# NJU-3DV/Relightable3DGaussian

Measured on AMD Instinct MI355X. Metric: train iters/s, synthetic lego-like 800x800, 300000 Gaussians (stage-2 hot path), higher is better.
Workload: dtype f32; 1 GPU; stage-2 train iteration (fused glue kernels + one-launch Adam): shading fwd/bwd (K=64) + rasterize fwd (S=16) + loss + rasterize bwd + Adam; 1 view/rank/step, 300000 Gaussians, 800x800, num_rendered~1755016; parallelism=dp1

## Files before the change

### relightable3dgaussian_amd/csrc/capi_rasterizer.hip

```cpp
#include "capi_internal.hpp"

#include <mutex>
#include <vector>

namespace r3dg {

GeometryLayout GeometryLayout::make(size_t P)
{
    GeometryLayout L;
    size_t o = 0;
    auto take = [&](size_t bytes) { size_t r = o; o = align_up(o + bytes, 256); return r; };
    L.depths = take(P * 4);
    L.clamped = take(P * 3);
    L.radii = take(P * 4);
    L.means2D = take(P * 8);
    L.cov3D = take(P * 24);
    L.conic_opacity = take(P * 16);
    L.rgb = take(P * 12);
    L.tiles_touched = take(P * 4);
    L.point_offsets = take(P * 4);
    L.block_sums = take(((P + 255) / 256 + 1) * 4);
    L.total = take(8);
    L.splat = take(P * 64);
    L.bytes = o;
// ... 96 lines not shown
        if (!g_ticket_pool.empty()) {
            ForwardTicket* t = g_ticket_pool.back();
            g_ticket_pool.pop_back();
            return t;
        }
    }
    ForwardTicket* t = new ForwardTicket();
    R3DG_HIP(hipEventCreateWithFlags(&t->ready, hipEventDisableTiming));
    R3DG_HIP(hipEventCreateWithFlags(&t->ordered, hipEventDisableTiming));
    R3DG_HIP(hipHostMalloc((void**)&t->host_total, sizeof(unsigned long long), hipHostMallocDefault));
    return t;
}
static void ticket_release(ForwardTicket* t)
{
    std::lock_guard<std::mutex> lk(g_ticket_mutex);
    g_ticket_pool.push_back(t);
}

static int enqueue_ordering(ForwardTicket* t, hipStream_t stream, int R)
{
    const ForwardArgs& a = t->a;
    const GeometryLayout& G = t->v.G;
    const ImageLayout& I = t->v.I;
    const bool debug = a.debug != 0;
    const int P = a.P, gx = t->v.gx, gy = t->v.gy, T = (int)t->v.T;
    char *gbuf = t->gbuf, *ibuf = t->ibuf;
    int* radii_p = t->radii_p;
    float* g_depths = (float*)(gbuf + G.depths);
    float* g_means2D = (float*)(gbuf + G.means2D);
    uint32_t* g_tiles = (uint32_t*)(gbuf + G.tiles_touched);
    uint32_t* g_block = (uint32_t*)(gbuf + G.block_sums);
    const bool direct = direct_binning_usable((long long)t->v.T);
    if (a.capacity >= 0 && !direct) {
        set_error("rasterize_forward (bounded): needs the direct tile binning and at most 16384 tiles: ask r3dg_bounded_forward_supported(width, height) first");
        return R3DG_EINVAL;
    }
    BinningLayout B = BinningLayout::make((size_t)R);
    char* bbuf = t->fused_front ? t->bbuf : (char*)a.binning_alloc(a.user, B.bytes);
    t->bbuf = bbuf;
    if (!bbuf) { set_error("rasterize_forward: binning resize callback returned NULL"); return R3DG_EALLOC; }
    uint64_t* keys_u = (uint64_t*)(bbuf + B.keys_unsorted);
    uint64_t* keys = (uint64_t*)(bbuf + B.keys);
    uint32_t* vals_u = (uint32_t*)(bbuf + B.vals_unsorted);
    uint32_t* vals = (uint32_t*)(bbuf + B.vals);
    t->point_list = vals;

    uint32_t* ranges = (uint32_t*)(ibuf + I.ranges);
    uint32_t* order = (uint32_t*)(ibuf + I.tile_order);
    uint32_t* big_list = (uint32_t*)(ibuf + I.big_list);
    uint32_t* big_count = (uint32_t*)(ibuf + I.big_count);
    if (direct) {
        uint32_t* tile_counts = (uint32_t*)(bbuf + B.sort_temp);
        StageTimer t_dup(stream, ST_DUPKEYS);
        launch_tile_binning(stream, P, T, g_means2D, g_depths, radii_p, g_tiles, g_block, gx, gy, tile_counts, tile_counts + T,
                            ranges, (uint32_t*)(gbuf + G.point_offsets), keys_u, (unsigned long long*)(gbuf + G.total), a.capacity,
                            a.overflow_flag, a.overflow_count, t->fused_front, order, tile_sort_small_cap(), big_list, big_count);
        check_launch(stream, debug, "tile_binning");
        t_dup.stop();
        StageTimer t_sort(stream, ST_SORT);
        if (!t->fused_front) {
            launch_tile_order(stream, T, ranges, order, tile_sort_small_cap(), big_list, big_count);
            check_launch(stream, debug, "tile_order");
        }
        launch_tile_sort(stream, T, order, ranges, big_list, big_count, keys, vals, keys_u, true);
        check_launch(stream, debug, "tile_sort");
        t_sort.stop();
        return R3DG_OK;
    }
    StageTimer t_dup(stream, ST_DUPKEYS);
    launch_duplicate_with_keys(stream, P, g_means2D, g_depths, g_tiles, g_block, (uint32_t*)(gbuf + G.point_offsets),
                               keys_u, vals_u, radii_p, gx, gy);
    check_launch(stream, debug, "duplicate_with_keys");
    t_dup.stop();
    const int bit = (int)higher_msb((uint32_t)T);
    StageTimer t_sort(stream, ST_SORT);
    if (opt(R3DG_OPT_TILE_BINNING)) {
        sort_pairs_range(stream, (size_t)R, keys_u, vals_u, keys, vals, 32, 32 + bit, bbuf + B.sort_temp, debug,
                         false);
        R3DG_HIP(hipMemsetAsync(ranges, 0, (size_t)T * 8, stream));
        launch_identify_tile_ranges(stream, R, keys, ranges);
        check_launch(stream, debug, "identify_tile_ranges");
        launch_tile_order(stream, T, ranges, order, tile_sort_small_cap(), big_list, big_count);
        check_launch(stream, debug, "tile_order");
        launch_tile_sort(stream, T, order, ranges, big_list, big_count, keys, vals, keys_u, false);
        check_launch(stream, debug, "tile_sort");
        t_sort.stop();
    } else {
        sort_pairs(stream, (size_t)R, keys_u, vals_u, keys, vals, 32 + bit, bbuf + B.sort_temp, debug);
        t_sort.stop();

        StageTimer t_rng(stream, ST_RANGES);
        R3DG_HIP(hipMemsetAsync(ranges, 0, (size_t)T * 8, stream));
        launch_identify_tile_ranges(stream, R, keys, ranges);
        check_launch(stream, debug, "identify_tile_ranges");
        t_rng.stop();
        if (opt(R3DG_OPT_TILE_ORDER)) {
            launch_tile_order(stream, T, ranges, order, 0u, nullptr, nullptr);
            check_launch(stream, debug, "tile_order");
        }
    }
    return R3DG_OK;
}

static void render_tiles(const ForwardTicket* t, hipStream_t stream)
{
    const ForwardArgs& a = t->a;
    const GeometryLayout& G = t->v.G;
    const ImageLayout& I = t->v.I;
    const bool debug = a.debug != 0;
    StageTimer t_rf(stream, ST_RENDER_FWD);
    launch_render_forward(stream, a.width, a.height, a.S,
                          opt(R3DG_OPT_TILE_ORDER) ? (uint32_t*)(t->ibuf + I.tile_order) : nullptr,
                          (uint32_t*)(t->ibuf + I.ranges), t->point_list, (const float*)(t->gbuf + G.splat), a.features,
                          (float*)(t->ibuf + I.final_T), (uint32_t*)(t->ibuf + I.n_contrib), a.background, a.out_color,
                          a.out_opacity, a.out_depth, a.out_feature, a.out_weights);
    check_launch(stream, debug, "render_forward");
// ... 387 lines not shown
```

### relightable3dgaussian_amd/csrc/launchers.hpp

```cpp
#pragma once
#include "common.hpp"

namespace r3dg {

__attribute__((visibility("hidden"))) int persistent_cus();

void release_gradient_records();
void launch_mark_visible(hipStream_t s, int P, const float* means3D, const float* vm, uint8_t* present);
void launch_preprocess(hipStream_t s, int P, int D, int M, const float* means3D, const float* scales, float scale_modifier,
                       const float* rotations, const float* opacities, const float* shs, uint8_t* clamped,
                       const float* cov3D_precomp, const float* colors_precomp, const float* vm, const float* pm,
                       const float* cam_pos, int W, int H, float tan_fovx, float tan_fovy, float focal_x, float focal_y,
                       int* radii, float* means2D, float* depths, float* cov3Ds, float* rgb, float* conic_opacity,
                       float* splat, int gx, int gy, uint32_t* tiles_touched, uint32_t* block_sums,
                       unsigned long long* total, bool scan_now, uint32_t* zero_words, int zero_n);
void launch_duplicate_with_keys(hipStream_t s, int P, const float* means2D, const float* depths,
                                const uint32_t* tiles_touched, const uint32_t* block_offsets, uint32_t* point_offsets,
                                uint64_t* keys, uint32_t* values, const int* radii, int gx, int gy);
void launch_identify_tile_ranges(hipStream_t s, int L, const uint64_t* keys, uint32_t* ranges);
void launch_tile_order(hipStream_t s, int T, const uint32_t* ranges, uint32_t* order, uint32_t small_cap, uint32_t* big_list,
                       uint32_t* big_count);
void launch_render_forward(hipStream_t s, int W, int H, int S, const uint32_t* tile_order, const uint32_t* ranges,
                           const uint32_t* point_list, const float* splat, const float* features, float* final_T,
                           uint32_t* n_contrib, const float* bg, float* out_color, float* out_opacity, float* out_depth,
// ... 110 lines not shown
                      float* dL_dpbr, float* dL_ddiffuse, float* block_absmax, float* light_l1_sum);
void launch_s2_activate_backward(hipStream_t s, int P, const float* xyz, const float* scaling_raw, const float* rotation_raw,
                                 const float* opacity_raw, const float* normal_raw, const float* base_raw,
                                 const float* rough_raw, const float* viewmatrix, const float* campos,
                                 const float* dL_dfeatures, const float* dL_dbase_shade, const float* dL_drough_shade,
                                 const float* dL_dviewdirs, const float* dL_dscales, const float* dL_drot,
                                 const float* dL_dopacity, const float* dL_dmeans3D, float* g_xyz, float* g_scaling,
                                 float* g_rotation, float* g_opacity, float* g_normal, float* g_base, float* g_rough, int He,
                                 int We, const float* env_raw, const float* env, float* dL_denv, float w_tv,
                                 float* g_env_raw, float* tv_sum, int consume);
void launch_s2_loss(hipStream_t s, int HW, const float* image, const float* opacity, const float* feature,
                    const float* pseudo_normal, const int* n_contrib, const float* gt, const float* bg,
                    const float* image_mask, float w_l1, float w_pbr, float w_normal, const float* extra_dimage,
                    const float* extra_dsrgb, float* dL_dimage, float* dL_dopacity, float* dL_dfeature, float* sums,
                    int sparse);
void launch_s2_smooth_forward(hipStream_t s, int W, int H, const float* opacity, const float* feature, const int* n_contrib,
                              const float* gt, const float* image_mask, float w_base, float w_rough, float w_light,
                              float* scratch, float* sums3);
void launch_s2_smooth_fused(hipStream_t s, int W, int H, const float* opacity, const float* feature, const int* n_contrib,
                            const float* gt, const float* image_mask, float w_base, float w_rough, float w_light,
                            int accumulate_normal, float* dL_dopacity, float* dL_dfeature, float* sums3);
void launch_s2_smooth_backward(hipStream_t s, int W, int H, const float* opacity, const float* feature, const int* n_contrib,
                               const float* image_mask, const float* scratch, int has_base, int has_rough, int has_light,
                               int accumulate_normal, float* dL_dopacity, float* dL_dfeature);
void launch_s2_pbr_srgb(hipStream_t s, int HW, const float* opacity, const float* feature, const int* n_contrib,
                        const float* bg, float* srgb);
void launch_s2_normals_srgb(hipStream_t s, int W, int H, const float* vm, float focal_x, float focal_y, float cx, float cy,
                            const float* opacity, const float* depths, float* normals, float* surface_xyz,
                            const float* feature, const int* n_contrib, const float* bg, float* srgb);
void launch_ssim_forward(hipStream_t s, int W, int H, int C, int n_images, const float* const* x, const float* y,
                         float* const* partials, float* const* sum);
void launch_ssim_backward(hipStream_t s, int W, int H, int C, int n_images, const float* const* x, const float* y,
                          float* const* partials, const float* scale, float* const* grad_x);
void launch_adam(hipStream_t s, int n_groups, const r3dg_adam_group* groups, float beta1, float beta2, float eps, int step,
                 float grad_scale, const float* skip_flag);
void launch_s1_pack(hipStream_t s, int P, const float* xyz, const float* viewmatrix, const float* normal, float* features);
void launch_s1_edge(hipStream_t s, int W, int H, const float* feature, const float* opacity, const int* n_contrib,
                    const float* gt, float* edge_g, float* sum_out);
void launch_s1_loss(hipStream_t s, int W, int H, const float* image, const float* opacity, const float* feature,
                    const float* pseudo_normal, const int* n_contrib, const float* gt, const float* image_mask, float w_l1,
                    float w_entropy, float w_normal, float w_smooth, float w_var, const float* extra_dimage,
                    const float* edge_g, float* dL_dimage, float* dL_dopacity, float* dL_dfeature, float* sums);
void launch_s1_activate_backward(hipStream_t s, int P, const float* xyz, const float* scaling_raw, const float* rotation_raw,
                                 const float* opacity_raw, const float* normal_raw, const float* viewmatrix,
                                 const float* dL_dfeatures, const float* dL_dscales, const float* dL_drot,
                                 const float* dL_dopacity, const float* dL_dmeans3D, float* g_xyz, float* g_scaling,
                                 float* g_rotation, float* g_opacity, float* g_normal);
void launch_s2_env_backward(hipStream_t s, int He, int We, const float* raw, const float* env, float* dL_denv, float w_tv,
                            float* g_raw, float* tv_sum, int consume);
uint32_t tile_sort_small_cap();
void launch_tile_sort(hipStream_t s, int T, const uint32_t* tile_order, const uint32_t* ranges, const uint32_t* big_list,
                      uint32_t* big_count, uint64_t* keys, uint32_t* vals, uint64_t* scratch, bool entries);
void launch_tile_binning(hipStream_t s, int P, int T, const float* means2D, const float* depths, const int* radii,
                         const uint32_t* tiles_touched, uint32_t* block_offsets, int gx, int gy, uint32_t* tile_counts,
                         uint32_t* cursor, uint32_t* ranges, uint32_t* point_offsets, uint64_t* entries,
                         unsigned long long* total, long long capacity, float* overflow_flag, unsigned int* overflow_count,
                         bool fused, uint32_t* order, uint32_t small_cap, uint32_t* big_list, uint32_t* big_count);
int tile_binning_max_tiles();
void launch_densify_accumulate(hipStream_t s, int P, const float* viewspace_grad, const float* normal_grad, const int* radii,
                               const float* weights, float* xyz_accum, float* normal_accum, float* denom,
                               float* weights_accum, float* max_radii2D, const float* skip_flag);
size_t densify_temp_bytes(size_t P);
void launch_densify_plan(hipStream_t s, int P, const r3dg_densify_config& cfg, const float* scaling_raw,
                         const float* opacity_raw, const float* xyz_accum, const float* normal_accum, const float* denom,
                         const float* weights_accum, const float* max_radii2D, int32_t* src_row, int32_t* kind,
                         int32_t* counts, void* temp);
void launch_densify_gather(hipStream_t s, int P_out, const int32_t* src_row, const int32_t* kind, int n_groups,
                           const r3dg_densify_group* groups, const float* xyz, const float* scaling_raw,
                           const float* rotation_raw, const float* normal_table, float split_divisor);
void launch_reset_opacity(hipStream_t s, int P, float cap, float* opacity_raw, float* exp_avg, float* exp_avg_sq);
void launch_relight_pack(hipStream_t s, int P, const float* xyz, const float* viewmatrix, const float* normal,
                         const float* base_color, const float* roughness, const float* shade_out, float* features);
void launch_relight_compose(hipStream_t s, int W, int H, float fx, float fy, float cx, float cy, const float* viewmatrix,
                            const float* tr, const float* env, int He, int We, const float* image, const float* opacity,
                            const float* feature, const int* n_contrib, float* pbr_env, float* render_env, float* env_only);
struct CaptureMaps {
    float *pbr, *base_color, *roughness, *normal, *visibility, *diffuse, *specular, *lights, *local_lights, *global_lights,
        *depth_var;
};
void launch_relight_capture(hipStream_t s, int W, int H, const float* feature, const float* opacity, const int* n_contrib,
                            const float* background, const float* mask, const CaptureMaps& maps);
void launch_eval_metric_tiles(hipStream_t s, int W, int H, int C, const float* pred, const float* gt, const float* mask,
                              const float* fill, int fill_is_image, double* tile_sums);
void launch_eval_image_metrics(hipStream_t s, int W, int H, int C, const float* pred, const float* gt, const float* mask,
                               const float* fill, int fill_is_image, double* tile_sums, double* row);
void launch_eval_median_ratio(hipStream_t s, int W, int H, const float* pred, const float* gt, const float* mask,
                              uint32_t* state, double* row);
size_t knn_temp_bytes(size_t P);
void knn_dist2(hipStream_t s, int P, const float* pts, float* dists, void* temp);
size_t bvh_build_temp_bytes(size_t P);
void bvh_build(hipStream_t s, int P, int32_t* nodes, float* aabbs, uint64_t* morton, void* temp);
void bvh_prepare_leaves(hipStream_t s, int P, const float* means, const float* scales, const float* rotations, int32_t* nodes,
                        float* aabbs, float* covs_inv);
void bvh_trace_count(hipStream_t s, int num_rays, const int32_t* nodes, const float* aabbs, const float* rays_o,
                     const float* rays_d, int32_t* counts, int* overflow);
void bvh_trace_fill(hipStream_t s, int num_rays, const int32_t* nodes, const float* aabbs, const float* rays_o,
                    const float* rays_d, const float* means, const int32_t* counts, const int64_t* offsets_inclusive,
                    uint64_t* keys, int32_t* points, float* positions, int32_t* ray_ids);
void bvh_trace_opacity(hipStream_t s, int num_rays, int P, const int32_t* nodes, const float* aabbs, const float* rays_o,
                       const float* rays_d, const float* means, const float* covs, const float* opac, const float* normals,
                       int32_t* contributes, float* out, int* overflow);
size_t bvh_trace_records_bytes(size_t P);
void bvh_pack_traversal(hipStream_t s, int P, const int32_t* nodes, const float* aabbs, const float* means,
                        const float* covs, const float* opac, const float* normals, void* records);
void bvh_trace_visits(hipStream_t s, int P, const void* records, unsigned long long out[2]);
void bvh_trace_opacity_packed(hipStream_t s, int num_rays, int P, void* records, const float* rays_o, const float* rays_d,
                              int32_t* contributes, float* out, int* overflow);
void bvh_trace_bundles(hipStream_t s, int P, int K, void* records, const int32_t* nodes, const float* zsamples, int leaf_lo,
                       int leaf_hi, float origin_offset, float* out, int32_t* contributes, float* dirs_out, int* overflow);
// ... 10 lines not shown
```

### relightable3dgaussian_amd/csrc/rasterizer_preprocess.hip

```cpp
#include <atomic>

#include "launchers.hpp"

namespace r3dg {

struct M3 {
    float c[3][3];
};
__device__ __forceinline__ M3 m3mul(const M3& A, const M3& B)
{
    M3 R;
#pragma unroll
    for (int j = 0; j < 3; j++)
#pragma unroll
        for (int i = 0; i < 3; i++)
            R.c[j][i] = A.c[0][i] * B.c[j][0] + A.c[1][i] * B.c[j][1] + A.c[2][i] * B.c[j][2];
    return R;
}
__device__ __forceinline__ M3 m3t(const M3& A)
{
    M3 R;
#pragma unroll
    for (int j = 0; j < 3; j++)
#pragma unroll
// ... 255 lines not shown
    if (live) {
        const float2 p = means2D[idx];
        tile_rect(p.x, p.y, radii[idx], gx, gy, x0, y0, x1, y1);
        dbits = __float_as_uint(depths[idx]);
    }
    const int w_rect = x1 - x0;
    const bool big = live && cnt > 32u;
    if (live && !big) {
        for (int y = y0; y < y1; y++)
            for (int x = x0; x < x1; x++) {
                uint64_t key = (uint64_t)(uint32_t)(y * gx + x);
                key = (key << 32) | dbits;
                keys[begin] = key;
                values[begin] = (uint32_t)idx;
                begin++;
            }
    }
    unsigned long long todo = __ballot(big);
    while (todo) {
        const int src = __ffsll((long long)todo) - 1;
        todo &= todo - 1;
        const int bx0 = __shfl(x0, src, 64), by0 = __shfl(y0, src, 64), bw = __shfl(w_rect, src, 64);
        const uint32_t bcnt = (uint32_t)__shfl((int)cnt, src, 64);
        const uint32_t bbegin = (uint32_t)__shfl((int)(end - cnt), src, 64);
        const uint32_t bbits = (uint32_t)__shfl((int)dbits, src, 64);
        const uint32_t bid = (uint32_t)(blockIdx.x * 256 + wave * 64 + src);
        for (uint32_t k = lane; k < bcnt; k += 64) {
            const int y = by0 + (int)(k / (uint32_t)bw), x = bx0 + (int)(k % (uint32_t)bw);
            uint64_t key = (uint64_t)(uint32_t)(y * gx + x);
            key = (key << 32) | bbits;
            keys[bbegin + k] = key;
            values[bbegin + k] = bid;
        }
    }
}

__global__ void identify_tile_ranges_kernel(int L, const uint64_t* __restrict__ keys, uint2* __restrict__ ranges)
{
    const int idx = blockIdx.x * blockDim.x + threadIdx.x;
    if (idx >= L) return;
    const uint32_t currtile = (uint32_t)(keys[idx] >> 32);
    if (idx == 0)
        ranges[currtile].x = 0;
    else {
        const uint32_t prevtile = (uint32_t)(keys[idx - 1] >> 32);
        if (currtile != prevtile) {
            ranges[prevtile].y = idx;
            ranges[currtile].x = idx;
        }
    }
    if (idx == L - 1) ranges[currtile].y = L;
}

__device__ __forceinline__ void tile_order_body(int T, const uint2* __restrict__ ranges, uint32_t* __restrict__ order,
                                                uint32_t small_cap, uint32_t* __restrict__ big_list,
                                                uint32_t* __restrict__ big_count)
{
    __shared__ uint32_t s_nbig;
    __shared__ uint32_t s_cnt[256];
    __shared__ uint32_t s_max;
    const int tid = threadIdx.x;
    if (tid < 256) s_cnt[tid] = 0;
    if (tid == 0) { s_max = 0; s_nbig = 0; }
    __syncthreads();
    uint32_t m = 0;
    for (int t = tid; t < T; t += 1024) {
        const uint32_t len = ranges[t].y - ranges[t].x;
        m = max(m, len);
        if (big_list != nullptr && len > small_cap) big_list[atomicAdd(&s_nbig, 1u)] = (uint32_t)t;
    }
    atomicMax(&s_max, m);
    __syncthreads();
    const uint32_t scale = s_max + 1;
    for (int t = tid; t < T; t += 1024) {
        const uint32_t len = ranges[t].y - ranges[t].x;
        const uint32_t cls = 255u - (uint32_t)(((uint64_t)len * 256u) / scale);
        atomicAdd(&s_cnt[cls], 1u);
    }
    __syncthreads();
    if (tid == 0) {
        uint32_t run = 0;
        for (int c = 0; c < 256; c++) {
            const uint32_t n = s_cnt[c];
            s_cnt[c] = run;
            run += n;
        }
    }
    __syncthreads();
    for (int t = tid; t < T; t += 1024) {
        const uint32_t len = ranges[t].y - ranges[t].x;
        const uint32_t cls = 255u - (uint32_t)(((uint64_t)len * 256u) / scale);
        order[atomicAdd(&s_cnt[cls], 1u)] = (uint32_t)t;
    }
    if (tid == 0 && big_count != nullptr) {
        big_count[0] = s_nbig;
        big_count[1] = 0;
    }
}

__global__ void __launch_bounds__(1024)
tile_order_kernel(int T, const uint2* __restrict__ ranges, uint32_t* __restrict__ order, uint32_t small_cap,
                  uint32_t* __restrict__ big_list, uint32_t* __restrict__ big_count)
{
    tile_order_body(T, ranges, order, small_cap, big_list, big_count);
}

constexpr int BIN_MAX_TILES = 16384;

constexpr int BIN_THREADS = 1024;
constexpr int BIN_MAX_ITERS = 4;

struct TileRect {
    int x0, y0, w, h;
};

__device__ __forceinline__ TileRect load_tile_rect(int idx, int P, const float2* __restrict__ means2D,
                                                   const int* __restrict__ radii, int gx, int gy)
{
    const int i = idx < P ? idx : P - 1;
    const int r = radii[i];
    const float2 p = means2D[i];
    TileRect t;
    int x0 = 0, y0 = 0, x1 = 0, y1 = 0;
    if (idx < P && r > 0) tile_rect(p.x, p.y, r, gx, gy, x0, y0, x1, y1);
    t.x0 = x0; t.y0 = y0; t.w = x1 - x0; t.h = y1 - y0;
    return t;
}

__device__ __forceinline__ int dealt_index_of(int it, int thread, int nb)
{
    const int q = (it * (BIN_THREADS / 64) + (thread >> 6)) * nb + (int)blockIdx.x;
    return q * 64 + (thread & 63);
}
__device__ __forceinline__ int dealt_index(int it, int nb) { return dealt_index_of(it, (int)threadIdx.x, nb); }

template <typename F>
__device__ __forceinline__ void small_rect_tiles(const TileRect& rc, int it, int idx, uint32_t payload, int gx, uint16_t* s_big,
                                                 uint32_t* s_nbig, F&& f)
{
    const uint32_t cnt = (uint32_t)(rc.w * rc.h);
    const bool big = cnt > 32u;
    if (cnt != 0u && !big) {
        int x = rc.x0, y = rc.y0;
        const int x1 = rc.x0 + rc.w;
        for (uint32_t k = 0; k < cnt; k++) {
            f((uint32_t)(y * gx + x), (uint32_t)idx, payload);
            if (++x == x1) {
                x = rc.x0;
                y++;
            }
        }
    }
    const unsigned long long m = __ballot(big);
    if (m) {
        const int lane = threadIdx.x & 63;
        uint32_t base = 0;
        if (lane == 0) base = atomicAdd(s_nbig, (uint32_t)__popcll(m));
        base = (uint32_t)__shfl((int)base, 0, 64);
        if (big) s_big[base + (uint32_t)__popcll(m & ((1ull << lane) - 1ull))] = (uint16_t)((it << 10) | (int)threadIdx.x);
    }
}

template <bool PAYLOAD_IS_DEPTH, typename F>
__device__ __forceinline__ void big_rect_tiles(const uint16_t* s_big, uint32_t n_big, int nb, const float2* __restrict__ means2D,
                                               const int* __restrict__ radii, const float* __restrict__ depths, int gx, int gy, F&& f)
{
    const int lane = threadIdx.x & 63;
    for (uint32_t r = threadIdx.x >> 6; r < n_big; r += BIN_THREADS / 64) {
        const int e = (int)s_big[r];
        const uint32_t g = (uint32_t)dealt_index_of(e >> 10, e & 1023, nb);
        const float2 p = means2D[g];
        int x0, y0, x1, y1;
        tile_rect(p.x, p.y, radii[g], gx, gy, x0, y0, x1, y1);
        const uint32_t pay = PAYLOAD_IS_DEPTH ? __float_as_uint(depths[g]) : 0u;
        const int w = x1 - x0;
        const uint32_t cnt = (uint32_t)(w * (y1 - y0));
        int y = y0 + lane / w, x = x0 + lane % w;
        const int dy = 64 / w, dx = 64 % w;
        for (uint32_t k = lane; k < cnt; k += 64) {
            f((uint32_t)(y * gx + x), g, pay);
            x += dx;
            y += dy;
            if (x >= x1) {
                x -= w;
                y++;
            }
        }
    }
}

__global__ void __launch_bounds__(BIN_THREADS)
tile_count_kernel(int P, int T, int iters, const float2* __restrict__ means2D, const int* __restrict__ radii, int gx, int gy,
                  uint32_t* __restrict__ tile_counts)
{
    extern __shared__ uint32_t s_bins[];
    uint16_t* s_big = reinterpret_cast<uint16_t*>(s_bins + T);
    __shared__ uint32_t s_nbig;
    const int nb = gridDim.x;
    TileRect rc[BIN_MAX_ITERS];
#pragma unroll
    for (int it = 0; it < BIN_MAX_ITERS; it++)
        rc[it] = load_tile_rect(it < iters ? dealt_index(it, nb) : P, P, means2D, radii, gx, gy);
    for (int t = threadIdx.x; t < T; t += BIN_THREADS) s_bins[t] = 0;
    if (threadIdx.x == 0) s_nbig = 0;
    __syncthreads();
    auto count = [&](uint32_t tile, uint32_t, uint32_t) { atomicAdd(&s_bins[tile], 1u); };
#pragma unroll
    for (int it = 0; it < BIN_MAX_ITERS; it++)
        if (it < iters) small_rect_tiles(rc[it], it, dealt_index(it, nb), 0u, gx, s_big, &s_nbig, count);
    __syncthreads();
    big_rect_tiles<false>(s_big, s_nbig, nb, means2D, radii, nullptr, gx, gy, count);
    __syncthreads();
    for (int t = threadIdx.x; t < T; t += BIN_THREADS) {
        const uint32_t c = s_bins[t];
        if (c) atomicAdd(&tile_counts[t], c);
    }
}

__global__ void __launch_bounds__(1024)
tile_scan_kernel(int T, const uint32_t* __restrict__ tile_counts, uint2* __restrict__ ranges, uint32_t* __restrict__ cursor,
                 unsigned long long* __restrict__ total, long long capacity, float* __restrict__ overflow_flag,
                 unsigned int* __restrict__ overflow_count, int nb_block_sums, uint32_t* __restrict__ block_sums)
{
    __shared__ uint32_t s_wave[16];
    __shared__ unsigned long long s_wave_b[16];
    const int tid = threadIdx.x, lane = tid & 63, wave = tid >> 6;
    const int per_t = (T + 1023) / 1024, t0 = tid * per_t, t1 = min(t0 + per_t, T);
    const int per_b = (nb_block_sums + 1023) / 1024, b0 = tid * per_b, b1 = min(b0 + per_b, nb_block_sums);
    uint32_t tsum = 0;
    for (int t = t0; t < t1; t++) tsum += tile_counts[t];
    unsigned long long bsum = 0;
    for (int b = b0; b < b1; b++) bsum += block_sums[b];
    const uint32_t tinc = wave_inclusive_scan_u32(tsum);
    unsigned long long binc = bsum;
    if (nb_block_sums > 0) {
#pragma unroll
        for (int o = 1; o < 64; o <<= 1) {
            const unsigned long long n = __shfl_up(binc, o, 64);
            if (lane >= o) binc += n;
        }
    }
    if (lane == 63) {
        s_wave[wave] = tinc;
        s_wave_b[wave] = binc;
    }
    __syncthreads();
    uint32_t toff = 0;
    unsigned long long boff = 0, count = 0;
    for (int w = 0; w < 16; w++) {
        if (w < wave) {
            toff += s_wave[w];
            boff += s_wave_b[w];
        }
        count += s_wave_b[w];
    }
    if (nb_block_sums > 0) {
        if (tid == 0) total[0] = count;
        unsigned long long run = boff + binc - bsum;
        for (int b = b0; b < b1; b++) {
            const uint32_t v = block_sums[b];
            block_sums[b] = (uint32_t)run;
            run += v;
        }
    } else {
        count = *total;
    }
    const bool over = capacity >= 0 && count > (unsigned long long)capacity;
    if (tid == 0 && overflow_flag != nullptr) *overflow_flag = over ? 1.0f : 0.0f;
    if (tid == 0 && over && overflow_count != nullptr) *overflow_count += 1u;
    uint32_t start = toff + tinc - tsum;
    for (int t = t0; t < t1; t++) {
        const uint32_t v = tile_counts[t];
        ranges[t] = (v && !over) ? make_uint2(start, start + v) : make_uint2(0u, 0u);
        cursor[t] = over ? 0u : start;
        start += v;
    }
}

__global__ void __launch_bounds__(BIN_THREADS)
tile_emit_kernel(int P, int T, int iters, const float2* __restrict__ means2D, const float* __restrict__ depths,
                 const int* __restrict__ radii, const uint32_t* __restrict__ tiles_touched,
                 const uint32_t* __restrict__ block_offsets, int gx, int gy, uint32_t* __restrict__ cursor,
                 uint32_t* __restrict__ point_offsets, uint64_t* __restrict__ entries,
                 const unsigned long long* __restrict__ total, long long capacity, int emit_blocks,
                 const uint2* __restrict__ ranges, uint32_t* __restrict__ order, uint32_t small_cap,
                 uint32_t* __restrict__ big_list, uint32_t* __restrict__ big_count)
{
    extern __shared__ uint32_t s_bins[];
    uint16_t* s_big = reinterpret_cast<uint16_t*>(s_bins + T);
    __shared__ uint32_t s_wave[BIN_MAX_ITERS][BIN_THREADS / 64];
    __shared__ uint32_t s_nbig;
    if ((int)blockIdx.x >= emit_blocks) {
        tile_order_body(T, ranges, order, small_cap, big_list, big_count);
        return;
    }
    const bool over = capacity >= 0 && *total > (unsigned long long)capacity;
    const int lane = threadIdx.x & 63, wave = threadIdx.x >> 6;
    for (int t = threadIdx.x; t < T; t += BIN_THREADS) s_bins[t] = 0;
    if (threadIdx.x == 0) s_nbig = 0;
    const int lin = blockIdx.x * iters * BIN_THREADS + threadIdx.x;
    uint32_t inc[BIN_MAX_ITERS], boff[BIN_MAX_ITERS], dbits[BIN_MAX_ITERS];
    TileRect rc[BIN_MAX_ITERS];
#pragma unroll
    for (int it = 0; it < BIN_MAX_ITERS; it++) {
        const int idx = it < iters ? dealt_index(it, emit_blocks) : P;
        rc[it] = load_tile_rect(idx, P, means2D, radii, gx, gy);
        dbits[it] = __float_as_uint(depths[idx < P ? idx : P - 1]);
    }
#pragma unroll
    for (int it = 0; it < BIN_MAX_ITERS; it++) {
        const int idx = lin + it * BIN_THREADS;
        const bool in = it < iters && idx < P;
        const uint32_t cnt = in ? tiles_touched[idx] : 0u;
        boff[it] = in ? block_offsets[idx >> 8] : 0u;
        inc[it] = wave_inclusive_scan_u32(cnt);
        if (lane == 63) s_wave[it][wave] = inc[it];
    }
    __syncthreads();
#pragma unroll
    for (int it = 0; it < BIN_MAX_ITERS; it++) {
        const int idx = lin + it * BIN_THREADS;
        if (it < iters && idx < P) {
            uint32_t off = boff[it];
            for (int w = wave & ~3; w < wave; w++) off += s_wave[it][w];
            point_offsets[idx] = off + inc[it];
        }
    }
    if (over) return;
    auto count = [&](uint32_t tile, uint32_t, uint32_t) { atomicAdd(&s_bins[tile], 1u); };
#pragma unroll
    for (int it = 0; it < BIN_MAX_ITERS; it++)
        if (it < iters) small_rect_tiles(rc[it], it, dealt_index(it, emit_blocks), 0u, gx, s_big, &s_nbig, count);
    __syncthreads();
    const uint32_t n_big = s_nbig;
    big_rect_tiles<false>(s_big, n_big, emit_blocks, means2D, radii, depths, gx, gy, count);
    __syncthreads();
    for (int t0 = threadIdx.x; t0 < T; t0 += 4 * BIN_THREADS) {
        uint32_t c[4], r[4];
#pragma unroll
        for (int k = 0; k < 4; k++) {
            const int t = t0 + k * BIN_THREADS;
            c[k] = t < T ? s_bins[t] : 0u;
        }
#pragma unroll
        for (int k = 0; k < 4; k++) r[k] = c[k] ? atomicAdd(&cursor[t0 + k * BIN_THREADS], c[k]) : 0u;
#pragma unroll
        for (int k = 0; k < 4; k++)
            if (c[k]) s_bins[t0 + k * BIN_THREADS] = r[k];
    }
    __syncthreads();
    auto emit = [&](uint32_t tile, uint32_t g, uint32_t depth_bits) {
        const uint32_t pos = atomicAdd(&s_bins[tile], 1u);
        entries[pos] = ((uint64_t)depth_bits << 32) | (uint64_t)g;
    };
#pragma unroll
    for (int it = 0; it < BIN_MAX_ITERS; it++)
        if (it < iters) {
            const TileRect& q = rc[it];
            const uint32_t cnt = (uint32_t)(q.w * q.h);
            if (cnt != 0u && cnt <= 32u) {
                int x = q.x0, y = q.y0;
                const int x1 = q.x0 + q.w;
                const uint32_t g = (uint32_t)dealt_index(it, emit_blocks);
                for (uint32_t k = 0; k < cnt; k++) {
                    emit((uint32_t)(y * gx + x), g, dbits[it]);
                    if (++x == x1) {
                        x = q.x0;
                        y++;
                    }
                }
            }
        }
    big_rect_tiles<true>(s_big, n_big, emit_blocks, means2D, radii, depths, gx, gy, emit);
}

void launch_tile_binning(hipStream_t s, int P, int T, const float* means2D, const float* depths, const int* radii,
                         const uint32_t* tiles_touched, uint32_t* block_offsets, int gx, int gy,
                         uint32_t* tile_counts , uint32_t* cursor , uint32_t* ranges,
                         uint32_t* point_offsets, uint64_t* entries, unsigned long long* total, long long capacity,
                         float* overflow_flag, unsigned int* overflow_count, bool fused, uint32_t* order, uint32_t small_cap,
                         uint32_t* big_list, uint32_t* big_count)
{
    if (!fused) R3DG_HIP(hipMemsetAsync(tile_counts, 0, (size_t)T * 4, s));
    const int iters = std::min(std::max(opt(R3DG_OPT_BINNING_BLOCK_K), 1), BIN_MAX_ITERS);
    const int per_block = iters * BIN_THREADS;
    const int nb = (P + per_block - 1) / per_block;
    const size_t smem = (size_t)T * 4 + (size_t)iters * BIN_THREADS * 2;
    if (smem + 1024 > 65536) {
        static std::atomic<unsigned long long> done{0};
        int dev = 0;
        R3DG_HIP(hipGetDevice(&dev));
        const unsigned long long bit = 1ull << (dev & 63);
        if (!(done.load(std::memory_order_acquire) & bit)) {
            const int want = BIN_MAX_TILES * 4 + BIN_MAX_ITERS * BIN_THREADS * 2;
            R3DG_HIP(hipFuncSetAttribute((const void*)tile_count_kernel, hipFuncAttributeMaxDynamicSharedMemorySize, want));
            R3DG_HIP(hipFuncSetAttribute((const void*)tile_emit_kernel, hipFuncAttributeMaxDynamicSharedMemorySize, want));
            done.fetch_or(bit, std::memory_order_release);
        }
    }
    tile_count_kernel<<<nb, BIN_THREADS, smem, s>>>(P, T, iters, (const float2*)means2D, radii, gx, gy, tile_counts);
    tile_scan_kernel<<<1, 1024, 0, s>>>(T, tile_counts, (uint2*)ranges, cursor, total, capacity, overflow_flag,
                                        overflow_count, fused ? (P + 255) / 256 : 0, block_offsets);
    tile_emit_kernel<<<nb + (fused ? 1 : 0), BIN_THREADS, smem, s>>>(
        P, T, iters, (const float2*)means2D, depths, radii, tiles_touched, block_offsets, gx, gy, cursor, point_offsets, entries,
        total, capacity, nb, (const uint2*)ranges, order, small_cap, big_list, big_count);
}

int tile_binning_max_tiles() { return BIN_MAX_TILES; }

void launch_tile_order(hipStream_t s, int T, const uint32_t* ranges, uint32_t* order, uint32_t small_cap,
                       uint32_t* big_list, uint32_t* big_count)
{
    tile_order_kernel<<<1, 1024, 0, s>>>(T, (const uint2*)ranges, order, small_cap, big_list, big_count);
}

void launch_mark_visible(hipStream_t s, int P, const float* means3D, const float* vm, uint8_t* present)
{
    if (P <= 0) return;
    mark_visible_kernel<<<(P + 255) / 256, 256, 0, s>>>(P, means3D, vm, present);
}

void launch_preprocess(hipStream_t s, int P, int D, int M, const float* means3D, const float* scales,
                       float scale_modifier, const float* rotations, const float* opacities, const float* shs,
                       uint8_t* clamped, const float* cov3D_precomp, const float* colors_precomp, const float* vm,
                       const float* pm, const float* cam_pos, int W, int H, float tan_fovx, float tan_fovy,
                       float focal_x, float focal_y, int* radii, float* means2D, float* depths, float* cov3Ds,
                       float* rgb, float* conic_opacity, float* splat, int gx, int gy, uint32_t* tiles_touched,
                       uint32_t* block_sums, unsigned long long* total, bool scan_now, uint32_t* zero_words, int zero_n)
{
    const int nb = (P + 255) / 256;
    if (zero_n > nb * 256) {
        R3DG_HIP(hipMemsetAsync(zero_words, 0, (size_t)zero_n * 4, s));
        zero_n = 0;
    }
    const bool staged = opt(R3DG_OPT_STAGE_SH_ROWS) && shs != nullptr && colors_precomp == nullptr && M >= 1 && M <= 16;
    if (staged)
        preprocess_kernel<true><<<nb, 256, 256 * ((3 * M) | 1) * sizeof(float), s>>>(
            P, D, M, means3D, scales, scale_modifier, rotations, opacities, shs, clamped, cov3D_precomp, colors_precomp,
            vm, pm, cam_pos, W, H, tan_fovx, tan_fovy, focal_x, focal_y, radii, (float2*)means2D, depths, cov3Ds, rgb,
            (float4*)conic_opacity, (float4*)splat, gx, gy, tiles_touched, block_sums, zero_words, zero_n);
    else
        preprocess_kernel<false><<<nb, 256, 0, s>>>(
            P, D, M, means3D, scales, scale_modifier, rotations, opacities, shs, clamped, cov3D_precomp, colors_precomp,
            vm, pm, cam_pos, W, H, tan_fovx, tan_fovy, focal_x, focal_y, radii, (float2*)means2D, depths, cov3Ds, rgb,
            (float4*)conic_opacity, (float4*)splat, gx, gy, tiles_touched, block_sums, zero_words, zero_n);
    if (scan_now) scan_block_sums_kernel<<<1, 1024, 0, s>>>(nb, block_sums, total);
}

void launch_duplicate_with_keys(hipStream_t s, int P, const float* means2D, const float* depths,
                                const uint32_t* tiles_touched, const uint32_t* block_offsets,
                                uint32_t* point_offsets, uint64_t* keys, uint32_t* values, const int* radii, int gx,
                                int gy)
{
    duplicate_with_keys_kernel<<<(P + 255) / 256, 256, 0, s>>>(P, (const float2*)means2D, depths, tiles_touched,
                                                             block_offsets, point_offsets, keys, values, radii, gx, gy);
}

void launch_identify_tile_ranges(hipStream_t s, int L, const uint64_t* keys, uint32_t* ranges)
// ... 7 lines not shown
```

Baseline: 823.6 iters/s.

## Fold tile scan and ordering into binning emit via per-block run offsets

The count kernel now records, for each block and tile, the atomic return value as a per-block run offset into a scratch buffer. The emit kernel then computes each tile's start with a block-local scan of tile counts, which removes the separate single-block tile_scan kernel and the second counting pass with cursor atomics in emit. Tile ordering is always done by an extra block in the emit launch, reading lengths from shared memory, so the separate tile_order launch is gone. In exchange it adds an nb×T scratch buffer of global writes and reads, and every emit block repeats the scan over all tile counts.

```diff
diff --git a/relightable3dgaussian_amd/csrc/capi_rasterizer.hip b/relightable3dgaussian_amd/csrc/capi_rasterizer.hip
--- a/relightable3dgaussian_amd/csrc/capi_rasterizer.hip
+++ b/relightable3dgaussian_amd/csrc/capi_rasterizer.hip
@@ -172,16 +172,12 @@
     if (direct) {
         uint32_t* tile_counts = (uint32_t*)(bbuf + B.sort_temp);
         StageTimer t_dup(stream, ST_DUPKEYS);
-        launch_tile_binning(stream, P, T, g_means2D, g_depths, radii_p, g_tiles, g_block, gx, gy, tile_counts, tile_counts + T,
-                            ranges, (uint32_t*)(gbuf + G.point_offsets), keys_u, (unsigned long long*)(gbuf + G.total), a.capacity,
+        launch_tile_binning(stream, P, T, g_means2D, g_depths, radii_p, g_tiles, g_block, gx, gy, tile_counts, ranges,
+                            (uint32_t*)(gbuf + G.point_offsets), keys_u, (unsigned long long*)(gbuf + G.total), a.capacity,
                             a.overflow_flag, a.overflow_count, t->fused_front, order, tile_sort_small_cap(), big_list, big_count);
         check_launch(stream, debug, "tile_binning");
         t_dup.stop();
         StageTimer t_sort(stream, ST_SORT);
-        if (!t->fused_front) {
-            launch_tile_order(stream, T, ranges, order, tile_sort_small_cap(), big_list, big_count);
-            check_launch(stream, debug, "tile_order");
-        }
         launch_tile_sort(stream, T, order, ranges, big_list, big_count, keys, vals, keys_u, true);
         check_launch(stream, debug, "tile_sort");
         t_sort.stop();
diff --git a/relightable3dgaussian_amd/csrc/launchers.hpp b/relightable3dgaussian_amd/csrc/launchers.hpp
--- a/relightable3dgaussian_amd/csrc/launchers.hpp
+++ b/relightable3dgaussian_amd/csrc/launchers.hpp
@@ -186,9 +186,8 @@
 void launch_tile_sort(hipStream_t s, int T, const uint32_t* tile_order, const uint32_t* ranges, const uint32_t* big_list,
                       uint32_t* big_count, uint64_t* keys, uint32_t* vals, uint64_t* scratch, bool entries);
 void launch_tile_binning(hipStream_t s, int P, int T, const float* means2D, const float* depths, const int* radii,
-                         const uint32_t* tiles_touched, uint32_t* block_offsets, int gx, int gy, uint32_t* tile_counts,
-                         uint32_t* cursor, uint32_t* ranges, uint32_t* point_offsets, uint64_t* entries,
-                         unsigned long long* total, long long capacity, float* overflow_flag, unsigned int* overflow_count,
+                         const uint32_t* tiles_touched, const uint32_t* block_sums, int gx, int gy, uint32_t* tile_counts,
+                         uint32_t* ranges, uint32_t* point_offsets, uint64_t* entries, unsigned long long* total, long long capacity, float* overflow_flag, unsigned int* overflow_count,
                          bool fused, uint32_t* order, uint32_t small_cap, uint32_t* big_list, uint32_t* big_count);
 int tile_binning_max_tiles();
 void launch_densify_accumulate(hipStream_t s, int P, const float* viewspace_grad, const float* normal_grad, const int* radii,
diff --git a/relightable3dgaussian_amd/csrc/rasterizer_preprocess.hip b/relightable3dgaussian_amd/csrc/rasterizer_preprocess.hip
--- a/relightable3dgaussian_amd/csrc/rasterizer_preprocess.hip
+++ b/relightable3dgaussian_amd/csrc/rasterizer_preprocess.hip
@@ -331,9 +331,9 @@
     if (idx == L - 1) ranges[currtile].y = L;
 }
 
-__device__ __forceinline__ void tile_order_body(int T, const uint2* __restrict__ ranges, uint32_t* __restrict__ order,
-                                                uint32_t small_cap, uint32_t* __restrict__ big_list,
-                                                uint32_t* __restrict__ big_count)
+template <typename LenOf>
+__device__ __forceinline__ void tile_order_body(int T, LenOf&& len_of, uint32_t* __restrict__ order, uint32_t small_cap,
+                                                uint32_t* __restrict__ big_list, uint32_t* __restrict__ big_count)
 {
     __shared__ uint32_t s_nbig;
     __shared__ uint32_t s_cnt[256];
@@ -344,7 +344,7 @@
     __syncthreads();
     uint32_t m = 0;
     for (int t = tid; t < T; t += 1024) {
-        const uint32_t len = ranges[t].y - ranges[t].x;
+        const uint32_t len = len_of(t);
         m = max(m, len);
         if (big_list != nullptr && len > small_cap) big_list[atomicAdd(&s_nbig, 1u)] = (uint32_t)t;
     }
@@ -352,7 +352,7 @@
     __syncthreads();
     const uint32_t scale = s_max + 1;
     for (int t = tid; t < T; t += 1024) {
-        const uint32_t len = ranges[t].y - ranges[t].x;
+        const uint32_t len = len_of(t);
         const uint32_t cls = 255u - (uint32_t)(((uint64_t)len * 256u) / scale);
         atomicAdd(&s_cnt[cls], 1u);
     }
@@ -367,7 +367,7 @@
     }
     __syncthreads();
     for (int t = tid; t < T; t += 1024) {
-        const uint32_t len = ranges[t].y - ranges[t].x;
+        const uint32_t len = len_of(t);
         const uint32_t cls = 255u - (uint32_t)(((uint64_t)len * 256u) / scale);
         order[atomicAdd(&s_cnt[cls], 1u)] = (uint32_t)t;
     }
@@ -381,7 +381,7 @@
 tile_order_kernel(int T, const uint2* __restrict__ ranges, uint32_t* __restrict__ order, uint32_t small_cap,
                   uint32_t* __restrict__ big_list, uint32_t* __restrict__ big_count)
 {
-    tile_order_body(T, ranges, order, small_cap, big_list, big_count);
+    tile_order_body(T, [&](int t) { return ranges[t].y - ranges[t].x; }, order, small_cap, big_list, big_count);
 }
 
 constexpr int BIN_MAX_TILES = 16384;
@@ -470,7 +470,7 @@
 
 __global__ void __launch_bounds__(BIN_THREADS)
 tile_count_kernel(int P, int T, int iters, const float2* __restrict__ means2D, const int* __restrict__ radii, int gx, int gy,
-                  uint32_t* __restrict__ tile_counts)
+                  uint32_t* __restrict__ tile_counts, uint32_t* __restrict__ run_offset )
 {
     extern __shared__ uint32_t s_bins[];
     uint16_t* s_big = reinterpret_cast<uint16_t*>(s_bins + T);
@@ -490,142 +490,144 @@
     __syncthreads();
     big_rect_tiles<false>(s_big, s_nbig, nb, means2D, radii, nullptr, gx, gy, count);
     __syncthreads();
-    for (int t = threadIdx.x; t < T; t += BIN_THREADS) {
-        const uint32_t c = s_bins[t];
-        if (c) atomicAdd(&tile_counts[t], c);
-    }
-}
-
-__global__ void __launch_bounds__(1024)
-tile_scan_kernel(int T, const uint32_t* __restrict__ tile_counts, uint2* __restrict__ ranges, uint32_t* __restrict__ cursor,
-                 unsigned long long* __restrict__ total, long long capacity, float* __restrict__ overflow_flag,
-                 unsigned int* __restrict__ overflow_count, int nb_block_sums, uint32_t* __restrict__ block_sums)
-{
-    __shared__ uint32_t s_wave[16];
-    __shared__ unsigned long long s_wave_b[16];
+    uint32_t* __restrict__ row = run_offset + (size_t)blockIdx.x * (size_t)T;
+    for (int t0 = threadIdx.x; t0 < T; t0 += 4 * BIN_THREADS) {
+        uint32_t c[4], r[4];
+#pragma unroll
+        for (int k = 0; k < 4; k++) {
+            const int t = t0 + k * BIN_THREADS;
+            c[k] = t < T ? s_bins[t] : 0u;
+        }
+#pragma unroll
+        for (int k = 0; k < 4; k++) r[k] = c[k] ? atomicAdd(&tile_counts[t0 + k * BIN_THREADS], c[k]) : 0u;
+#pragma unroll
+        for (int k = 0; k < 4; k++)
+            if (t0 + k * BIN_THREADS < T) row[t0 + k * BIN_THREADS] = r[k];
+    }
+}
+
+struct TileScan {
+    int t0, t1;
+    uint32_t start;
+    unsigned long long total;
+    unsigned long long sums_front;
+};
+
+__device__ __forceinline__ TileScan scan_tile_counts(int T, const uint32_t* __restrict__ tile_counts, bool scan_sums, int n_front,
+                                                     const uint32_t* __restrict__ block_sums)
+{
+    __shared__ uint32_t s_scan_t[BIN_THREADS / 64];
+    __shared__ unsigned long long s_scan_b[BIN_THREADS / 64];
     const int tid = threadIdx.x, lane = tid & 63, wave = tid >> 6;
-    const int per_t = (T + 1023) / 1024, t0 = tid * per_t, t1 = min(t0 + per_t, T);
-    const int per_b = (nb_block_sums + 1023) / 1024, b0 = tid * per_b, b1 = min(b0 + per_b, nb_block_sums);
+    const int per_t = (T + BIN_THREADS - 1) / BIN_THREADS;
+    TileScan r;
+    r.t0 = min(tid * per_t, T);
+    r.t1 = min(r.t0 + per_t, T);
     uint32_t tsum = 0;
-    for (int t = t0; t < t1; t++) tsum += tile_counts[t];
+    for (int t = r.t0; t < r.t1; t++) tsum += tile_counts[t];
     unsigned long long bsum = 0;
-    for (int b = b0; b < b1; b++) bsum += block_sums[b];
+    if (scan_sums)
+        for (int b = tid; b < n_front; b += BIN_THREADS) bsum += block_sums[b];
     const uint32_t tinc = wave_inclusive_scan_u32(tsum);
-    unsigned long long binc = bsum;
-    if (nb_block_sums > 0) {
-#pragma unroll
-        for (int o = 1; o < 64; o <<= 1) {
-            const unsigned long long n = __shfl_up(binc, o, 64);
-            if (lane >= o) binc += n;
-        }
-    }
-    if (lane == 63) {
-        s_wave[wave] = tinc;
-        s_wave_b[wave] = binc;
-    }
+    if (scan_sums) {
+#pragma unroll
+        for (int o = 32; o > 0; o >>= 1) bsum += __shfl_xor(bsum, o, 64);
+    }
+    if (lane == 63) s_scan_t[wave] = tinc;
+    if (lane == 0) s_scan_b[wave] = bsum;
     __syncthreads();
     uint32_t toff = 0;
-    unsigned long long boff = 0, count = 0;
-    for (int w = 0; w < 16; w++) {
-        if (w < wave) {
-            toff += s_wave[w];
-            boff += s_wave_b[w];
-        }
-        count += s_wave_b[w];
-    }
-    if (nb_block_sums > 0) {
-        if (tid == 0) total[0] = count;
-        unsigned long long run = boff + binc - bsum;
-        for (int b = b0; b < b1; b++) {
-            const uint32_t v = block_sums[b];
-            block_sums[b] = (uint32_t)run;
-            run += v;
-        }
-    } else {
-        count = *total;
-    }
-    const bool over = capacity >= 0 && count > (unsigned long long)capacity;
-    if (tid == 0 && overflow_flag != nullptr) *overflow_flag = over ? 1.0f : 0.0f;
-    if (tid == 0 && over && overflow_count != nullptr) *overflow_count += 1u;
-    uint32_t start = toff + tinc - tsum;
-    for (int t = t0; t < t1; t++) {
-        const uint32_t v = tile_counts[t];
-        ranges[t] = (v && !over) ? make_uint2(start, start + v) : make_uint2(0u, 0u);
-        cursor[t] = over ? 0u : start;
-        start += v;
-    }
+    r.total = 0;
+    r.sums_front = 0;
+    for (int w = 0; w < BIN_THREADS / 64; w++) {
+        if (w < wave) toff += s_scan_t[w];
+        r.total += s_scan_t[w];
+        r.sums_front += s_scan_b[w];
+    }
+    r.start = toff + tinc - tsum;
+    return r;
 }
 
 __global__ void __launch_bounds__(BIN_THREADS)
 tile_emit_kernel(int P, int T, int iters, const float2* __restrict__ means2D, const float* __restrict__ depths,
                  const int* __restrict__ radii, const uint32_t* __restrict__ tiles_touched,
-                 const uint32_t* __restrict__ block_offsets, int gx, int gy, uint32_t* __restrict__ cursor,
+                 const uint32_t* __restrict__ block_sums, bool scan_sums, int gx, int gy,
+                 const uint32_t* __restrict__ tile_counts, const uint32_t* __restrict__ run_offset,
                  uint32_t* __restrict__ point_offsets, uint64_t* __restrict__ entries,
-                 const unsigned long long* __restrict__ total, long long capacity, int emit_blocks,
-                 const uint2* __restrict__ ranges, uint32_t* __restrict__ order, uint32_t small_cap,
-                 uint32_t* __restrict__ big_list, uint32_t* __restrict__ big_count)
+                 unsigned long long* __restrict__ total, long long capacity, float* __restrict__ overflow_flag,
+                 unsigned int* __restrict__ overflow_count, int emit_blocks, uint2* __restrict__ ranges,
+                 uint32_t* __restrict__ order, uint32_t small_cap, uint32_t* __restrict__ big_list,
+                 uint32_t* __restrict__ big_count)
 {
     extern __shared__ uint32_t s_bins[];
     uint16_t* s_big = reinterpret_cast<uint16_t*>(s_bins + T);
     __shared__ uint32_t s_wave[BIN_MAX_ITERS][BIN_THREADS / 64];
     __shared__ uint32_t s_nbig;
-    if ((int)blockIdx.x >= emit_blocks) {
-        tile_order_body(T, ranges, order, small_cap, big_list, big_count);
+    const bool order_block = (int)blockIdx.x >= emit_blocks;
+    const int lane = threadIdx.x & 63, wave = threadIdx.x >> 6;
+    const int lin = blockIdx.x * iters * BIN_THREADS + threadIdx.x;
+    const int first_chunk = blockIdx.x * iters * (BIN_THREADS / 256);
+    uint32_t inc[BIN_MAX_ITERS], dbits[BIN_MAX_ITERS];
+    TileRect rc[BIN_MAX_ITERS];
+    uint32_t front = 0;
+    if (!order_block) {
+#pragma unroll
+        for (int it = 0; it < BIN_MAX_ITERS; it++) {
+            const int idx = it < iters ? dealt_index(it, emit_blocks) : P;
+            rc[it] = load_tile_rect(idx, P, means2D, radii, gx, gy);
+            dbits[it] = __float_as_uint(depths[idx < P ? idx : P - 1]);
+        }
+        if (!scan_sums) front = block_sums[first_chunk];
+#pragma unroll
+        for (int it = 0; it < BIN_MAX_ITERS; it++) {
+            const int idx = lin + it * BIN_THREADS;
+            const uint32_t cnt = it < iters && idx < P ? tiles_touched[idx] : 0u;
+            inc[it] = wave_inclusive_scan_u32(cnt);
+            if (lane == 63) s_wave[it][wave] = inc[it];
+        }
+        if (threadIdx.x == 0) s_nbig = 0;
+    }
+    const TileScan sc = scan_tile_counts(T, tile_counts, scan_sums && !order_block, first_chunk, block_sums);
+    const bool over = capacity >= 0 && sc.total > (unsigned long long)capacity;
+    if (order_block) {
+        uint32_t start = sc.start;
+        for (int t = sc.t0; t < sc.t1; t++) {
+            const uint32_t v = tile_counts[t];
+            ranges[t] = (v && !over) ? make_uint2(start, start + v) : make_uint2(0u, 0u);
+            s_bins[t] = over ? 0u : v;
+            start += v;
+        }
+        if (threadIdx.x == 0) {
+            if (scan_sums) *total = sc.total;
+            if (overflow_flag != nullptr) *overflow_flag = over ? 1.0f : 0.0f;
+            if (over && overflow_count != nullptr) *overflow_count += 1u;
+        }
+        __syncthreads();
+        tile_order_body(T, [&](int t) { return s_bins[t]; }, order, small_cap, big_list, big_count);
         return;
     }
-    const bool over = capacity >= 0 && *total > (unsigned long long)capacity;
-    const int lane = threadIdx.x & 63, wave = threadIdx.x >> 6;
-    for (int t = threadIdx.x; t < T; t += BIN_THREADS) s_bins[t] = 0;
-    if (threadIdx.x == 0) s_nbig = 0;
-    const int lin = blockIdx.x * iters * BIN_THREADS + threadIdx.x;
-    uint32_t inc[BIN_MAX_ITERS], boff[BIN_MAX_ITERS], dbits[BIN_MAX_ITERS];
-    TileRect rc[BIN_MAX_ITERS];
+    if (scan_sums) front = (uint32_t)sc.sums_front;
 #pragma unroll
     for (int it = 0; it < BIN_MAX_ITERS; it++) {
-        const int idx = it < iters ? dealt_index(it, emit_blocks) : P;
-        rc[it] = load_tile_rect(idx, P, means2D, radii, gx, gy);
-        dbits[it] = __float_as_uint(depths[idx < P ? idx : P - 1]);
-    }
-#pragma unroll
-    for (int it = 0; it < BIN_MAX_ITERS; it++) {
-        const int idx = lin + it * BIN_THREADS;
-        const bool in = it < iters && idx < P;
-        const uint32_t cnt = in ? tiles_touched[idx] : 0u;
-        boff[it] = in ? block_offsets[idx >> 8] : 0u;
-        inc[it] = wave_inclusive_scan_u32(cnt);
-        if (lane == 63) s_wave[it][wave] = inc[it];
-    }
-    __syncthreads();
-#pragma unroll
-    for (int it = 0; it < BIN_MAX_ITERS; it++) {
-        const int idx = lin + it * BIN_THREADS;
-        if (it < iters && idx < P) {
-            uint32_t off = boff[it];
-            for (int w = wave & ~3; w < wave; w++) off += s_wave[it][w];
-            point_offsets[idx] = off + inc[it];
+        if (it < iters) {
+            const int idx = lin + it * BIN_THREADS;
+            uint32_t off = front;
+            for (int w = 0; w < BIN_THREADS / 64; w++) {
+                const uint32_t n = s_wave[it][w];
+                if (w < wave) off += n;
+                front += n;
+            }
+            if (idx < P) point_offsets[idx] = off + inc[it];
         }
     }
     if (over) return;
-    auto count = [&](uint32_t tile, uint32_t, uint32_t) { atomicAdd(&s_bins[tile], 1u); };
-#pragma unroll
-    for (int it = 0; it < BIN_MAX_ITERS; it++)
-        if (it < iters) small_rect_tiles(rc[it], it, dealt_index(it, emit_blocks), 0u, gx, s_big, &s_nbig, count);
-    __syncthreads();
-    const uint32_t n_big = s_nbig;
-    big_rect_tiles<false>(s_big, n_big, emit_blocks, means2D, radii, depths, gx, gy, count);
-    __syncthreads();
-    for (int t0 = threadIdx.x; t0 < T; t0 += 4 * BIN_THREADS) {
-        uint32_t c[4], r[4];
-#pragma unroll
-        for (int k = 0; k < 4; k++) {
-            const int t = t0 + k * BIN_THREADS;
-            c[k] = t < T ? s_bins[t] : 0u;
-        }
-#pragma unroll
-        for (int k = 0; k < 4; k++) r[k] = c[k] ? atomicAdd(&cursor[t0 + k * BIN_THREADS], c[k]) : 0u;
-#pragma unroll
-        for (int k = 0; k < 4; k++)
-            if (c[k]) s_bins[t0 + k * BIN_THREADS] = r[k];
+    {
+        const uint32_t* __restrict__ row = run_offset + (size_t)blockIdx.x * (size_t)T;
+        uint32_t start = sc.start;
+        for (int t = sc.t0; t < sc.t1; t++) {
+            s_bins[t] = start + row[t];
+            start += tile_counts[t];
+        }
     }
     __syncthreads();
     auto emit = [&](uint32_t tile, uint32_t g, uint32_t depth_bits) {
@@ -634,38 +636,24 @@
     };
 #pragma unroll
     for (int it = 0; it < BIN_MAX_ITERS; it++)
-        if (it < iters) {
-            const TileRect& q = rc[it];
-            const uint32_t cnt = (uint32_t)(q.w * q.h);
-            if (cnt != 0u && cnt <= 32u) {
-                int x = q.x0, y = q.y0;
-                const int x1 = q.x0 + q.w;
-                const uint32_t g = (uint32_t)dealt_index(it, emit_blocks);
-                for (uint32_t k = 0; k < cnt; k++) {
-                    emit((uint32_t)(y * gx + x), g, dbits[it]);
-                    if (++x == x1) {
-                        x = q.x0;
-                        y++;
-                    }
-                }
-            }
-        }
-    big_rect_tiles<true>(s_big, n_big, emit_blocks, means2D, radii, depths, gx, gy, emit);
+        if (it < iters) small_rect_tiles(rc[it], it, dealt_index(it, emit_blocks), dbits[it], gx, s_big, &s_nbig, emit);
+    __syncthreads();
+    big_rect_tiles<true>(s_big, s_nbig, emit_blocks, means2D, radii, depths, gx, gy, emit);
 }
 
 void launch_tile_binning(hipStream_t s, int P, int T, const float* means2D, const float* depths, const int* radii,
-                         const uint32_t* tiles_touched, uint32_t* block_offsets, int gx, int gy,
-                         uint32_t* tile_counts , uint32_t* cursor , uint32_t* ranges,
-                         uint32_t* point_offsets, uint64_t* entries, unsigned long long* total, long long capacity,
-                         float* overflow_flag, unsigned int* overflow_count, bool fused, uint32_t* order, uint32_t small_cap,
-                         uint32_t* big_list, uint32_t* big_count)
+                         const uint32_t* tiles_touched, const uint32_t* block_sums, int gx, int gy,
+                         uint32_t* tile_counts , uint32_t* ranges, uint32_t* point_offsets, uint64_t* entries,
+                         unsigned long long* total, long long capacity, float* overflow_flag, unsigned int* overflow_count,
+                         bool fused, uint32_t* order, uint32_t small_cap, uint32_t* big_list, uint32_t* big_count)
 {
     if (!fused) R3DG_HIP(hipMemsetAsync(tile_counts, 0, (size_t)T * 4, s));
     const int iters = std::min(std::max(opt(R3DG_OPT_BINNING_BLOCK_K), 1), BIN_MAX_ITERS);
     const int per_block = iters * BIN_THREADS;
     const int nb = (P + per_block - 1) / per_block;
+    uint32_t* run_offset = (uint32_t*)stream_scratch(s, 3, (size_t)nb * (size_t)T * 4);
     const size_t smem = (size_t)T * 4 + (size_t)iters * BIN_THREADS * 2;
-    if (smem + 1024 > 65536) {
+    if (smem + 2048 > 65536) {
         static std::atomic<unsigned long long> done{0};
         int dev = 0;
         R3DG_HIP(hipGetDevice(&dev));
@@ -677,12 +665,11 @@
             done.fetch_or(bit, std::memory_order_release);
         }
     }
-    tile_count_kernel<<<nb, BIN_THREADS, smem, s>>>(P, T, iters, (const float2*)means2D, radii, gx, gy, tile_counts);
-    tile_scan_kernel<<<1, 1024, 0, s>>>(T, tile_counts, (uint2*)ranges, cursor, total, capacity, overflow_flag,
-                                        overflow_count, fused ? (P + 255) / 256 : 0, block_offsets);
-    tile_emit_kernel<<<nb + (fused ? 1 : 0), BIN_THREADS, smem, s>>>(
-        P, T, iters, (const float2*)means2D, depths, radii, tiles_touched, block_offsets, gx, gy, cursor, point_offsets, entries,
-        total, capacity, nb, (const uint2*)ranges, order, small_cap, big_list, big_count);
+    tile_count_kernel<<<nb, BIN_THREADS, smem, s>>>(P, T, iters, (const float2*)means2D, radii, gx, gy, tile_counts, run_offset);
+    tile_emit_kernel<<<nb + 1, BIN_THREADS, smem, s>>>(
+        P, T, iters, (const float2*)means2D, depths, radii, tiles_touched, block_sums, fused, gx, gy, tile_counts, run_offset,
+        point_offsets, entries, total, capacity, overflow_flag, overflow_count, nb, (uint2*)ranges, order, small_cap, big_list,
+        big_count);
 }
 
 int tile_binning_max_tiles() { return BIN_MAX_TILES; }
```

Result: no change. 823.0 iters/s (-0.1%).
